# barbararoessle/e2e_multi_view_matching

Hardware: NVIDIA H100
Metric: view-tuples/sec @1024 kpts 5-view (higher is better)
Workload: dtype f32 via split operands on the tensor cores (fp16x3 / tf32x3, fp32-faithful) / f64 pose kernels

## Files before the change

e2e_multi_view_matching_b200/csrc/gemm_tc.cu:

```cuda
#include <cstring>
#include <map>
#include <mutex>
#include <tuple>
#include <cuda_fp16.h>
#include "common.cuh"
#include "kernels.cuh"
#include "tc_common.cuh"

namespace {

constexpr int BM = 128;
constexpr int PRODUCER_WARP = 8;
constexpr int NTHREADS = 384;
constexpr int PRODUCER_REGS = 40, CONSUMER_REGS = 232;
enum { W_RAW = 0, W_TF32 = 1, W_F16 = 2 };

template <int BN, int NPASS, int WM>
struct Cfg {
  static constexpr int BK = WM == W_F16 ? 64 : 32;
  static constexpr int A_BYTES = BM * BK * 4;
  static constexpr int W_PLANE = BN * 128;
  static constexpr int PLANES = NPASS == 3 ? 2 : 1;
  static constexpr int STAGE_BYTES = A_BYTES + PLANES * W_PLANE;
  static constexpr int TMA_BYTES = A_BYTES + (WM == W_RAW ? 1 : PLANES) * W_PLANE;
  static constexpr int STAGES = (196608 / STAGE_BYTES) < 6 ? (196608 / STAGE_BYTES) : 6;
  static constexpr bool STAGED = BN == 128 && NPASS == 3 && WM != W_RAW;
  static constexpr int OUT_BYTES = STAGED ? 2 * 16384 : 0;
  static constexpr int SMEM_BYTES = STAGES * STAGE_BYTES + OUT_BYTES + 1024  + 256 ;
  static_assert(SMEM_BYTES <= 232448, "over the sm_90 dynamic shared memory opt-in limit");
};

struct GArgs {
  const float* bias;
  const float* R; int ldr;
  float* C; int ldc;
  int M, N, K, K1;
  float alpha;
  int relu;
  float* VT; int vt_col0; int n_pad;
  float* KLO; float* VTLO;
  __half* KH16; __half* KL16; __half* VH16; __half* VL16;
  int tiles_m, tiles_n;
  int ksplit;
  int stage;
};

struct StoreMaps {
  CUtensorMap c, r, p[4];
};

struct ScoreTab {
  int n_pairs, batch, n_views, n_pad;
  int a[MVM_MAX_PAIRS], b[MVM_MAX_PAIRS], m[MVM_MAX_PAIRS], n[MVM_MAX_PAIRS];
  float* scores[MVM_MAX_PAIRS];
};

__device__ __forceinline__ float tf32_hi(float x) {
  return __uint_as_float((__float_as_uint(x) + 0x1000u) & 0xffffe000u);
}
__device__ __forceinline__ void split_pack_h(float x0, float x1, uint32_t& hi, uint32_t& lo) {
  const __half2 h = __floats2half2_rn(x0, x1);
  const float2 hf = __half22float2(h);
  const __half2 l = __floats2half2_rn(x0 - hf.x, x1 - hf.y);
  hi = *reinterpret_cast<const uint32_t*>(&h);
  lo = *reinterpret_cast<const uint32_t*>(&l);
}
__device__ __forceinline__ void sts_f2(uint32_t a, float2 v) {
  asm volatile("st.shared.v2.f32 [%0], {%1, %2};" ::"r"(a), "f"(v.x), "f"(v.y) : "memory");
}
__device__ __forceinline__ void sts_u32(uint32_t a, uint32_t v) {
  asm volatile("st.shared.b32 [%0], %1;" ::"r"(a), "r"(v) : "memory");
}
__device__ __forceinline__ float2 lds_f2(uint32_t a) {
  float2 v;
  asm volatile("ld.shared.v2.f32 {%0, %1}, [%2];" : "=f"(v.x), "=f"(v.y) : "r"(a) : "memory");
  return v;
}
__device__ __forceinline__ void fence_afrag(uint32_t (&a)[4][4]) {
#pragma unroll
  for (int i = 0; i < 4; ++i)
#pragma unroll
    for (int e = 0; e < 4; ++e) asm volatile("" : "+r"(a[i][e])::"memory");
}

template <int BN, int NPASS, int WM, bool SCORE>
__global__ void __launch_bounds__(NTHREADS, 1)
gemm_wg_kernel(const __grid_constant__ CUtensorMap tmA, const __grid_constant__ CUtensorMap tmA2,
               const __grid_constant__ CUtensorMap tmWhi, const __grid_constant__ CUtensorMap tmWlo,
               const __grid_constant__ GArgs g, const __grid_constant__ ScoreTab st,
               const __grid_constant__ StoreMaps sm) {
  using C_ = Cfg<BN, NPASS, WM>;
  static_assert(NPASS == 3 || WM == W_RAW, "single pass reads the raw W");
  constexpr int BK = C_::BK, STAGES = C_::STAGES, A_BYTES = C_::A_BYTES, W_PLANE = C_::W_PLANE;
  constexpr int STAGE_BYTES = C_::STAGE_BYTES;
  constexpr int KSTEPS = 4;
  constexpr bool PIPE = BN == 128;
  constexpr bool STAGED = C_::STAGED && !SCORE;
  extern __shared__ uint8_t smem_raw[];
  uint8_t* smem = reinterpret_cast<uint8_t*>((reinterpret_cast<uintptr_t>(smem_raw) + 1023) & ~uintptr_t(1023));
  uint8_t* obuf = smem + STAGES * STAGE_BYTES;
  uint64_t* full = reinterpret_cast<uint64_t*>(obuf + C_::OUT_BYTES);
  uint64_t* empty = full + STAGES;
  uint64_t* ostaged = empty + STAGES;
  uint64_t* ofree = ostaged + 2;

  const int warp = threadIdx.x >> 5, lane = threadIdx.x & 31;
  const int nk = SCORE ? g.K / BK : g.K / BK / g.ksplit;
  const int per_prob = g.tiles_m * g.tiles_n;
  const int n_tiles = SCORE ? per_prob * st.n_pairs * st.batch : per_prob * g.ksplit;
  auto decode = [&](int tile, int& m0, int& n0, int& a_row, int& w_row, int& prob) {
    prob = tile / per_prob;
    const int r = tile % per_prob;
    m0 = (r / g.tiles_n) * BM; n0 = (r % g.tiles_n) * BN;
    if (!SCORE) {
      a_row = m0; w_row = n0;
    } else {
      const int p = prob / st.batch, bi = prob % st.batch;
      a_row = (bi * st.n_views + st.a[p]) * st.n_pad + m0;
      w_row = (bi * st.n_views + st.b[p]) * st.n_pad + n0;
    }
  };
  auto tile_kind = [&](int n0) {
    if (g.VT && n0 >= g.vt_col0) return -1;
    if (g.KH16 && n0 >= 256) return 1;
    if (g.KLO && n0 >= 256 && n0 < 512) return 2;
    return 0;
  };

  if (threadIdx.x == 0) {
    for (int s = 0; s < STAGES; ++s) {
      tc::mbar_init(full + s, 1);
      tc::mbar_init(empty + s, 256);
    }
    if (STAGED)
      for (int b = 0; b < 2; ++b) {
        tc::mbar_init(ostaged + b, 256);
        tc::mbar_init(ofree + b, 1);
      }
    tc::fence_barrier_init();
  }
  __syncthreads();

  if (warp >= PRODUCER_WARP) {
    asm volatile("setmaxnreg.dec.sync.aligned.u32 %0;" ::"n"(PRODUCER_REGS));
    if (STAGED && g.stage && warp == PRODUCER_WARP + 1 && lane == 0) {
      tc::prefetch_tmap(&sm.c);
      if (g.R) tc::prefetch_tmap(&sm.r);
      if (g.KH16)
        for (int i = 0; i < 4; ++i) tc::prefetch_tmap(&sm.p[i]);
      if (g.KLO) tc::prefetch_tmap(&sm.p[0]);
      auto hand_back = [&](uint32_t u, int tile, int q) {
        uint64_t* bar = ofree + (u & 1);
        if (!g.R) {
          tc::mbar_arrive(bar);
        } else if (tile < n_tiles) {
          int m0, n0, a_row, w_row, prob;
          decode(tile, m0, n0, a_row, w_row, prob);
          tc::mbar_arrive_expect_tx(bar, 16384);
          tc::tma_load_2d(obuf + (u & 1) * 16384, &sm.r, bar, n0 + 32 * q, m0);
        }
      };
      hand_back(0, blockIdx.x, 0);
      hand_back(1, blockIdx.x, 1);
      uint32_t u = 0;
      for (int tile = blockIdx.x; tile < n_tiles; tile += gridDim.x) {
        int m0, n0, a_row, w_row, prob;
        decode(tile, m0, n0, a_row, w_row, prob);
        const int kind = tile_kind(n0);
        if (kind < 0) continue;
        const int rounds = kind == 2 ? 8 : 4;
        for (int j = 0; j < rounds; ++j, ++u) {
          const uint8_t* buf = obuf + (u & 1) * 16384;
          tc::mbar_wait(ostaged + (u & 1), (u >> 1) & 1);
          if (kind == 0) {
            tc::tma_store_2d(&sm.c, buf, n0 + 32 * j, m0 + prob * g.tiles_m * BM);
          } else if (kind == 1) {
            const bool v = n0 >= 512;
            tc::tma_store_2d(&sm.p[(v ? 2 : 0) + (j & 1)], buf, n0 - (v ? 512 : 256) + 64 * (j >> 1), m0);
          } else {
            if (j & 1) tc::tma_store_2d(&sm.p[0], buf, n0 - 256 + 32 * (j >> 1), m0);
            else tc::tma_store_2d(&sm.c, buf, n0 + 32 * (j >> 1), m0);
          }
          tc::tma_store_commit();
          tc::tma_store_wait_read<0>();
          hand_back(u + 2, j < 2 ? tile : tile + gridDim.x, (j + 2) & 3);
        }
      }
      tc::tma_store_wait_all();
    }
    if (warp == PRODUCER_WARP && lane == 0) {
      tc::prefetch_tmap(&tmA); tc::prefetch_tmap(&tmA2); tc::prefetch_tmap(&tmWhi); tc::prefetch_tmap(&tmWlo);
      uint32_t it = 0;
      for (int tile = blockIdx.x; tile < n_tiles; tile += gridDim.x) {
        int m0, n0, a_row, w_row, prob;
        decode(tile, m0, n0, a_row, w_row, prob);
        for (int kt = 0; kt < nk; ++kt, ++it) {
          const int s = it % STAGES;
          tc::mbar_wait(empty + s, ((it / STAGES) & 1) ^ 1);
          tc::mbar_arrive_expect_tx(full + s, C_::TMA_BYTES);
          uint8_t* sp = smem + s * STAGE_BYTES;
          const int k = kt * BK + (SCORE ? 0 : prob * nk * BK);
          if (k < g.K1) tc::tma_load_2d(sp, &tmA, full + s, k, a_row);
          else tc::tma_load_2d(sp, &tmA2, full + s, k - g.K1, a_row);
          if (WM == W_F16) {
            if (k < g.K1) tc::tma_load_2d(sp + 16384, &tmA, full + s, k + 32, a_row);
            else tc::tma_load_2d(sp + 16384, &tmA2, full + s, k + 32 - g.K1, a_row);
          }
          tc::tma_load_2d(sp + A_BYTES, &tmWhi, full + s, k, w_row);
          if (WM != W_RAW) tc::tma_load_2d(sp + A_BYTES + W_PLANE, &tmWlo, full + s, k, w_row);
        }
      }
    }
    return;
  }

  asm volatile("setmaxnreg.inc.sync.aligned.u32 %0;" ::"n"(CONSUMER_REGS));
  const int wg = warp >> 2, wq = warp & 3;
  const int gr = lane >> 2, tq = lane & 3;
  const int row0 = wg * 64 + wq * 16 + gr;
  float acc[BN / 2];
  uint32_t ahi0[KSTEPS][4], alo0[KSTEPS][4], ahi1[KSTEPS][4], alo1[KSTEPS][4];

  auto prep = [&](uint32_t it, uint32_t (&ahi)[KSTEPS][4], uint32_t (&alo)[KSTEPS][4]) {
      const int s = it % STAGES;
      tc::mbar_wait(full + s, (it / STAGES) & 1);
      uint8_t* sp = smem + s * STAGE_BYTES;
      if (WM == W_RAW && NPASS == 3) {
        float4* w = reinterpret_cast<float4*>(sp + A_BYTES);
        float4* wl = reinterpret_cast<float4*>(sp + A_BYTES + W_PLANE);
#pragma unroll 4
        for (int i = threadIdx.x; i < BN * 32 / 4; i += 256) {
          const float4 x = w[i];
          float4 h;
          h.x = tc::tf32_rn(x.x); h.y = tc::tf32_rn(x.y); h.z = tc::tf32_rn(x.z); h.w = tc::tf32_rn(x.w);
          w[i] = h;
          wl[i] = make_float4(tc::tf32_rn(x.x - h.x), tc::tf32_rn(x.y - h.y), tc::tf32_rn(x.z - h.z), tc::tf32_rn(x.w - h.w));
        }
// ... 3 lines not shown
      const uint8_t* ar = sp + row0 * 128;
#pragma unroll
      for (int kk = 0; kk < KSTEPS; ++kk) {
        if (WM == W_F16) {
          const uint8_t* ab = ar + (kk >> 1) * 16384;
          const int ch = 4 * (kk & 1) + (tq >> 1), wo = (tq & 1) * 8;
          const float2 x0 = *reinterpret_cast<const float2*>(ab + ((ch ^ gr) << 4) + wo);
          const float2 x1 = *reinterpret_cast<const float2*>(ab + 1024 + ((ch ^ gr) << 4) + wo);
          const float2 x2 = *reinterpret_cast<const float2*>(ab + (((ch + 2) ^ gr) << 4) + wo);
          const float2 x3 = *reinterpret_cast<const float2*>(ab + 1024 + (((ch + 2) ^ gr) << 4) + wo);
          split_pack_h(x0.x, x0.y, ahi[kk][0], alo[kk][0]);
          split_pack_h(x1.x, x1.y, ahi[kk][1], alo[kk][1]);
          split_pack_h(x2.x, x2.y, ahi[kk][2], alo[kk][2]);
          split_pack_h(x3.x, x3.y, ahi[kk][3], alo[kk][3]);
        } else {
          float x[4];
          x[0] = *reinterpret_cast<const float*>(ar + (((2 * kk) ^ gr) << 4) + tq * 4);
          x[1] = *reinterpret_cast<const float*>(ar + 1024 + (((2 * kk) ^ gr) << 4) + tq * 4);
          x[2] = *reinterpret_cast<const float*>(ar + (((2 * kk + 1) ^ gr) << 4) + tq * 4);
          x[3] = *reinterpret_cast<const float*>(ar + 1024 + (((2 * kk + 1) ^ gr) << 4) + tq * 4);
#pragma unroll
          for (int e = 0; e < 4; ++e) {
            if (NPASS == 3) {
              const float h = tf32_hi(x[e]);
              ahi[kk][e] = __float_as_uint(h);
              alo[kk][e] = __float_as_uint(tf32_hi(x[e] - h));
            } else {
              ahi[kk][e] = __float_as_uint(x[e]);
            }
          }
        }
      }
  };
  auto issue = [&](uint32_t it, const uint32_t (&ahi)[KSTEPS][4], const uint32_t (&alo)[KSTEPS][4]) {
      const uint32_t whi = tc::smem_u32(smem + (it % STAGES) * STAGE_BYTES + A_BYTES);
      tc::wgmma_fence();
#pragma unroll
      for (int kk = 0; kk < KSTEPS; ++kk) {
#pragma unroll
        for (int nh = 0; nh < BN / 128; ++nh) {
          float* d = acc + nh * 64;
          const uint32_t wb = whi + nh * 16384 + kk * 32;
          if (WM == W_F16) {
            tc::wgmma_f16_rs<128, 0>(d, ahi[kk], tc::make_sw128_desc(wb));
            tc::wgmma_f16_rs<128, 0>(d, ahi[kk], tc::make_sw128_desc(wb + W_PLANE));
            tc::wgmma_f16_rs<128, 0>(d, alo[kk], tc::make_sw128_desc(wb));
          } else {
            tc::wgmma_tf32_rs<128>(d, ahi[kk], tc::make_sw128_desc(wb));
            if (NPASS == 3) {
              tc::wgmma_tf32_rs<128>(d, ahi[kk], tc::make_sw128_desc(wb + W_PLANE));
              tc::wgmma_tf32_rs<128>(d, alo[kk], tc::make_sw128_desc(wb));
            }
          }
        }
      }
      tc::wgmma_commit();
  };
  auto keep = [&](uint32_t (&ahi)[KSTEPS][4], uint32_t (&alo)[KSTEPS][4]) {
    fence_afrag(ahi);
    if (NPASS == 3) fence_afrag(alo);
  };

  auto stage_round = [&](uint32_t u, int n0, int i0, int ni, int mode, int plane) {
    const uint32_t buf = tc::smem_u32(obuf + (u & 1) * 16384);
    float2 bv[8];
#pragma unroll
    for (int c = 0; c < ni; ++c) {
      const int n = n0 + 8 * (i0 + c) + 2 * tq;
      bv[c] = g.bias ? make_float2(__ldg(g.bias + n), __ldg(g.bias + n + 1)) : make_float2(0.f, 0.f);
    }
    tc::mbar_wait(ofree + (u & 1), (u >> 1) & 1);
#pragma unroll
    for (int c = 0; c < ni; ++c) {
      const int i = i0 + c;
#pragma unroll
      for (int hh = 0; hh < 2; ++hh) {
        const int r = row0 + 8 * hh;
        float x0 = __fmul_rn(g.alpha, acc[4 * i + 2 * hh]), x1 = __fmul_rn(g.alpha, acc[4 * i + 2 * hh + 1]);
        if (g.bias) { x0 = __fadd_rn(x0, bv[c].x); x1 = __fadd_rn(x1, bv[c].y); }
// ... 50 lines not shown
        prep(it + kt, ahi0, alo0);
        issue(it + kt, ahi0, alo0);
        tc::wgmma_wait<0>();
        tc::fence_acc<BN>(acc);
        keep(ahi0, alo0);
        tc::mbar_arrive(empty + (it + kt) % STAGES);
      }
    }
    it += nk;

    if (SCORE) {
      const int p = prob / st.batch, bi = prob % st.batch;
      const int pm = st.m[p], pn = st.n[p];
      float* Cp = st.scores[p] + (long long)bi * (pm + 1) * (pn + 1);
#pragma unroll
      for (int hh = 0; hh < 2; ++hh) {
        const int gm = m0 + row0 + 8 * hh;
        if (gm >= pm) continue;
#pragma unroll
        for (int i = 0; i < BN / 8; ++i) {
          const int gn = n0 + 8 * i + 2 * tq;
          if (gn < pn) Cp[(long long)gm * (pn + 1) + gn] = g.alpha * acc[4 * i + 2 * hh];
          if (gn + 1 < pn) Cp[(long long)gm * (pn + 1) + gn + 1] = g.alpha * acc[4 * i + 2 * hh + 1];
        }
      }
      continue;
    }
    if constexpr (STAGED) {
      const int kind = g.stage ? tile_kind(n0) : -1;
      if (kind >= 0) {
#pragma unroll
        for (int j = 0; j < 8; ++j) {
          if (kind == 1) {
            if (j < 4) stage_round(u + j, n0, 8 * (j >> 1), 8, 1, j & 1);
          } else if (kind == 2) {
            stage_round(u + j, n0, 4 * (j >> 1), 4, 2, j & 1);
          } else if (j < 4) {
            stage_round(u + j, n0, 4 * j, 4, 0, 0);
          }
        }
        u += kind == 2 ? 8 : 4;
        continue;
      }
    }
    auto put = [&](int m, int n, float x0, float x1) {
      if (g.VT && n >= g.vt_col0) {
        const int slab = m / g.n_pad, ii = m % g.n_pad;
        const long long off = ((long long)slab * (g.N - g.vt_col0) + (n - g.vt_col0)) * g.n_pad + ii;
        if (g.VTLO) {
          const float h0 = tf32_hi(x0), h1 = tf32_hi(x1);
          g.VT[off] = h0; g.VT[off + g.n_pad] = h1;
          g.VTLO[off] = tf32_hi(x0 - h0); g.VTLO[off + g.n_pad] = tf32_hi(x1 - h1);
        } else {
          g.VT[off] = x0; g.VT[off + g.n_pad] = x1;
        }
      } else if (g.KH16 && n >= 256) {
        const bool is_v = n >= 512;
        const long long o = (long long)m * 256 + n - (is_v ? 512 : 256);
        uint32_t hi, lo;
        split_pack_h(x0, x1, hi, lo);
        *reinterpret_cast<uint32_t*>((is_v ? g.VH16 : g.KH16) + o) = hi;
        *reinterpret_cast<uint32_t*>((is_v ? g.VL16 : g.KL16) + o) = lo;
      } else if (g.KLO && n >= 256 && n < 512) {
        const float h0 = tf32_hi(x0), h1 = tf32_hi(x1);
        *reinterpret_cast<float2*>(g.C + (long long)m * g.ldc + n) = make_float2(h0, h1);
        *reinterpret_cast<float2*>(g.KLO + (long long)m * 256 + n - 256) = make_float2(tf32_hi(x0 - h0), tf32_hi(x1 - h1));
      } else {
        const long long c_row = m + (long long)prob * g.tiles_m * BM;
        *reinterpret_cast<float2*>(g.C + c_row * g.ldc + n) = make_float2(x0, x1);
      }
    };
    if constexpr (PIPE) {
      constexpr int ICH = 8;
#pragma unroll
// ... 15 lines not shown
          const int i = i0 + c, n = n0 + 8 * i + 2 * tq;
#pragma unroll
          for (int hh = 0; hh < 2; ++hh) {
            const int m = m0 + row0 + 8 * hh;
            if (m >= g.M) continue;
            float x0 = g.alpha * acc[4 * i + 2 * hh], x1 = g.alpha * acc[4 * i + 2 * hh + 1];
            if (g.bias) { x0 += bv[c].x; x1 += bv[c].y; }
            if (g.relu) { x0 = fmaxf(x0, 0.f); x1 = fmaxf(x1, 0.f); }
            if (g.R) { x0 += rv[c][hh].x; x1 += rv[c][hh].y; }
            put(m, n, x0, x1);
          }
        }
      }
    } else {
#pragma unroll
      for (int hh = 0; hh < 2; ++hh) {
        const int m = m0 + row0 + 8 * hh;
        if (m >= g.M) continue;
#pragma unroll
        for (int i = 0; i < BN / 8; ++i) {
          const int n = n0 + 8 * i + 2 * tq;
          float x0 = g.alpha * acc[4 * i + 2 * hh], x1 = g.alpha * acc[4 * i + 2 * hh + 1];
          if (g.bias) { x0 += __ldg(g.bias + n); x1 += __ldg(g.bias + n + 1); }
          if (g.relu) { x0 = fmaxf(x0, 0.f); x1 = fmaxf(x1, 0.f); }
          if (g.R) {
            const float2 r = __ldg(reinterpret_cast<const float2*>(g.R + (long long)m * g.ldr + n));
            x0 += r.x; x1 += r.y;
          }
          put(m, n, x0, x1);
        }
      }
    }
  }
}

template <int BN, int NPASS, int WM, bool SCORE>
int launch_wg(const CUtensorMap* tA, const CUtensorMap* tA2, const CUtensorMap* tWhi, const CUtensorMap* tWlo,
              const GArgs& g, const ScoreTab& st, long long n_tiles, bool persistent, cudaStream_t stream,
              const StoreMaps& sm) {
  using C_ = Cfg<BN, NPASS, WM>;
  if (!tA || !tA2 || !tWhi || !tWlo) return MVM_ERR_LAUNCH;
  if (n_tiles <= 0) return MVM_OK;
  if (cudaFuncSetAttribute(gemm_wg_kernel<BN, NPASS, WM, SCORE>, cudaFuncAttributeMaxDynamicSharedMemorySize,
                           C_::SMEM_BYTES) != cudaSuccess)
    return MVM_ERR_LAUNCH;
  const int n_sm = mvm_dev_info().n_sm;
  const int grid = (persistent && n_tiles > n_sm) ? n_sm : (int)n_tiles;
  gemm_wg_kernel<BN, NPASS, WM, SCORE><<<grid, NTHREADS, C_::SMEM_BYTES, stream>>>(*tA, *tA2, *tWhi, *tWlo, g, st, sm);
  MVM_CHECK_LAUNCH();
  return MVM_OK;
}

StoreMaps no_store_maps() {
  StoreMaps none;
  memset(&none, 0, sizeof(none));
  return none;
}

GArgs make_args(const GemmDesc& d, float* VT, int vt_col0, int n_pad, float* KLO, float* VTLO, int bn) {
  GArgs g;
  memset(&g, 0, sizeof(g));
  g.bias = d.bias; g.R = d.R; g.ldr = d.ldr; g.C = d.C; g.ldc = d.ldc; g.M = d.M; g.N = d.N; g.K = d.K;
  g.K1 = d.K1; g.alpha = d.alpha; g.relu = d.relu; g.VT = VT; g.vt_col0 = vt_col0; g.n_pad = n_pad;
  g.KLO = KLO; g.VTLO = VTLO;
  g.tiles_m = mvm_div_up(d.M, BM); g.tiles_n = d.N / bn; g.ksplit = 1;
  return g;
// ... 61 lines not shown

}

const CUtensorMap* mvm_get_tmap_3d(const float* base, long long slabs, long long rows, long long cols,
                                   long long ld_row, long long ld_slab, int box_rows) {
  std::lock_guard<std::mutex> lk(g_tmap_mu);
  TmKey key(base, slabs, rows, cols, ld_row, ld_slab, box_rows);
  auto it = g_tmaps.find(key);
  if (it != g_tmaps.end()) return it->second;
  EncodeFn enc = get_encode();
  if (!enc) return nullptr;
  CUtensorMap* tm = new CUtensorMap;
  const int rank = slabs > 0 ? 3 : 2;
  cuuint64_t dims[3] = {(cuuint64_t)cols, (cuuint64_t)rows, (cuuint64_t)(slabs > 0 ? slabs : 1)};
  cuuint64_t strides[2] = {(cuuint64_t)ld_row * 4, (cuuint64_t)ld_slab * 4};
  cuuint32_t box[3] = {32, (cuuint32_t)box_rows, 1};
  cuuint32_t estr[3] = {1, 1, 1};
  CUresult r = enc(tm, CU_TENSOR_MAP_DATA_TYPE_FLOAT32, rank, const_cast<float*>(base), dims, strides, box, estr,
                   CU_TENSOR_MAP_INTERLEAVE_NONE, CU_TENSOR_MAP_SWIZZLE_128B, CU_TENSOR_MAP_L2_PROMOTION_L2_128B,
                   CU_TENSOR_MAP_FLOAT_OOB_FILL_NONE);
  if (r != CUDA_SUCCESS) {
    fprintf(stderr, "[mvm_b200] cuTensorMapEncodeTiled failed (%d) rows=%lld cols=%lld ld=%lld\n", (int)r, rows, cols, ld_row);
    delete tm;
    return nullptr;
  }
  g_tmaps[key] = tm;
  return tm;
}

const CUtensorMap* mvm_get_tmap_2d(const float* base, long long rows, long long cols, long long ld, int box_rows) {
  return mvm_get_tmap_3d(base, 0, rows, cols, ld, 0, box_rows);
}

const CUtensorMap* mvm_get_tmap_2d_f16(const void* base, long long rows, long long cols, long long ld, int box_rows) {
  std::lock_guard<std::mutex> lk(g_tmap_mu);
  TmKey key(base, -16, rows, cols, ld, 0, box_rows);
  auto it = g_tmaps.find(key);
  if (it != g_tmaps.end()) return it->second;
  EncodeFn enc = get_encode();
  if (!enc) return nullptr;
  CUtensorMap* tm = new CUtensorMap;
  cuuint64_t dims[2] = {(cuuint64_t)cols, (cuuint64_t)rows};
  cuuint64_t strides[1] = {(cuuint64_t)ld * 2};
  cuuint32_t box[2] = {64, (cuuint32_t)box_rows};
  cuuint32_t estr[2] = {1, 1};
  CUresult r = enc(tm, CU_TENSOR_MAP_DATA_TYPE_FLOAT16, 2, const_cast<void*>(base), dims, strides, box, estr,
                   CU_TENSOR_MAP_INTERLEAVE_NONE, CU_TENSOR_MAP_SWIZZLE_128B, CU_TENSOR_MAP_L2_PROMOTION_L2_128B,
                   CU_TENSOR_MAP_FLOAT_OOB_FILL_NONE);
  if (r != CUDA_SUCCESS) {
    fprintf(stderr, "[mvm_b200] cuTensorMapEncodeTiled (f16) failed (%d) rows=%lld cols=%lld ld=%lld\n", (int)r, rows, cols, ld);
    delete tm;
    return nullptr;
  }
  g_tmaps[key] = tm;
  return tm;
}


int g_gemm_bn = 256;
extern "C" void mvm_debug_set_gemm_tile(int bn) { g_gemm_bn = bn == 256 ? 256 : 128; }
int g_gemm_persist = 1;
extern "C" void mvm_debug_set_gemm_kernel(int persistent) { g_gemm_persist = persistent ? 1 : 0; }

int mvm_default_gemm_tile() { return g_gemm_bn; }
int mvm_default_gemm_persistent() { return g_gemm_persist; }

int launch_gemm_tc(const GemmDesc& d, int n_pass, float* VT, int vt_col0, int n_pad, cudaStream_t stream,
                   float* KLO, float* VTLO, int gemm_tile, int gemm_persist) {
  if (gemm_tile < 0) gemm_tile = g_gemm_bn;
  if (gemm_persist < 0) gemm_persist = g_gemm_persist;
  MVM_REQUIRE(gemm_desc_valid(d, GEMM_TC_TF32));
  MVM_REQUIRE(d.W || (n_pass == 3 && d.Whi && d.Wlo));
  MVM_REQUIRE(mvm_aligned(KLO, 8));
  MvmProfScope prof__(MVM_TAG_GEMM, stream);
  if (gemm_persist && n_pass == 3 && d.Whi && d.Wlo) return launch_gemm_tc_persist(d, VT, vt_col0, n_pad, KLO, VTLO, stream);
  if (gemm_tile == 256 && d.N % 256 == 0) {
    if (n_pass == 3 && d.Whi && d.Wlo) return launch_cfg<256, 3, W_TF32>(d, VT, vt_col0, n_pad, KLO, VTLO, false, stream);
    if (n_pass == 1) return launch_cfg<256, 1, W_RAW>(d, VT, vt_col0, n_pad, nullptr, nullptr, false, stream);
  }
  if (n_pass == 3 && d.Whi && d.Wlo) return launch_cfg<128, 3, W_TF32>(d, VT, vt_col0, n_pad, KLO, VTLO, false, stream);
  if (n_pass == 3) return launch_cfg<128, 3, W_RAW>(d, VT, vt_col0, n_pad, KLO, VTLO, false, stream);
  return launch_cfg<128, 1, W_RAW>(d, VT, vt_col0, n_pad, nullptr, nullptr, false, stream);
}

int launch_gemm_tc_persist(const GemmDesc& d, float* VT, int vt_col0, int n_pad, float* KLO, float* VTLO,
                           cudaStream_t stream, const HalfPlanes* hp, int ksplit, float* slabs) {
  MVM_REQUIRE(ksplit >= 1 && (ksplit == 1 || (slabs && d.M % BM == 0 && d.K % (32 * ksplit) == 0 && !d.Whi16 && !d.bias && !d.R && !d.A2 &&
                                               !d.relu && !VT && !KLO && !hp)));
  const bool f16 = d.Whi16 != nullptr && d.Wlo16 != nullptr && d.K % 64 == 0 && d.K1 % 64 == 0 && d.wscale > 0.f;
  MVM_REQUIRE(f16 ? gemm_desc_valid(d, GEMM_TC_F16) : gemm_desc_valid(d, GEMM_TC_TF32) && d.Whi && d.Wlo);
  MVM_REQUIRE(mvm_aligned(KLO, 8) && mvm_aligned(slabs, 16));
  MVM_REQUIRE(!hp || (mvm_aligned(hp->kh, 4) && mvm_aligned(hp->kl, 4) && mvm_aligned(hp->vh, 4) && mvm_aligned(hp->vl, 4)));
  const CUtensorMap* tA = mvm_get_tmap_2d(d.A, d.M, d.K1, d.lda, BM);
  const CUtensorMap* tA2 = d.A2 ? mvm_get_tmap_2d(d.A2, d.M, d.K - d.K1, d.lda2, BM) : tA;
  GArgs g = make_args(d, VT, vt_col0, n_pad, KLO, VTLO, 128);
  if (ksplit > 1) { g.C = slabs; g.ldc = d.N; }
  g.ksplit = ksplit;
  if (hp) {
    g.KH16 = (__half*)hp->kh; g.KL16 = (__half*)hp->kl; g.VH16 = (__half*)hp->vh; g.VL16 = (__half*)hp->vl;
  }
  const long long n_tiles = (long long)g.tiles_m * g.tiles_n * ksplit;
  StoreMaps sm = no_store_maps();
  const void* planes[4] = {g.KH16, g.KL16, g.VH16, g.VL16};
  bool stage = mvm_aligned(g.C, 16) && mvm_aligned(g.R, 16) && mvm_aligned(g.KLO, 16) && (!g.VT || g.vt_col0 % 128 == 0) &&
               (!g.R || (!g.KH16 && !g.KLO && !g.VT));
  for (const void* p : planes) stage = stage && mvm_aligned(p, 16);
  if (stage) {
    const CUtensorMap* c = mvm_get_tmap_2d(g.C, (long long)(ksplit - 1) * g.tiles_m * BM + g.M, g.N, g.ldc, BM);
    const CUtensorMap* r = g.R ? mvm_get_tmap_2d(g.R, g.M, g.N, g.ldr, BM) : c;
    if (!c || !r) return MVM_ERR_LAUNCH;
    sm.c = *c; sm.r = *r;
    for (int i = 0; i < 4; ++i) {
      const CUtensorMap* p = g.KH16 ? mvm_get_tmap_2d_f16(planes[i], g.M, 256, 256, BM)
                                    : g.KLO && i == 0 ? mvm_get_tmap_2d(g.KLO, g.M, 256, 256, BM) : c;
      if (!p) return MVM_ERR_LAUNCH;
      sm.p[i] = *p;
    }
    g.stage = 1;
  }
  if (f16) {
    g.alpha = d.alpha / d.wscale;
    const CUtensorMap* tWhi = mvm_get_tmap_2d_f16(d.Whi16, d.N, d.K, d.ldw, 128);
    const CUtensorMap* tWlo = mvm_get_tmap_2d_f16(d.Wlo16, d.N, d.K, d.ldw, 128);
    return launch_wg<128, 3, W_F16, false>(tA, tA2, tWhi, tWlo, g, no_scores(), n_tiles, true, stream, sm);
  }
  const CUtensorMap* tWhi = mvm_get_tmap_2d(d.Whi, d.N, d.K, d.ldw, 128);
  const CUtensorMap* tWlo = mvm_get_tmap_2d(d.Wlo, d.N, d.K, d.ldw, 128);
  return launch_wg<128, 3, W_TF32, false>(tA, tA2, tWhi, tWlo, g, no_scores(), n_tiles, true, stream, sm);
}

int launch_splitk_reduce(const float* slabs, float* C, int M, int N, int ldc, int ksplit, cudaStream_t stream) {
  MVM_REQUIRE(N % 4 == 0 && ldc % 4 == 0 && mvm_aligned(slabs, 16) && mvm_aligned(C, 16));
  const long long n = (long long)M * (N / 4);
  splitk_reduce_kernel<<<(unsigned)((n + 255) / 256), 256, 0, stream>>>(reinterpret_cast<const float4*>(slabs), C, M, N / 4, ldc, ksplit);
  MVM_CHECK_LAUNCH();
  return MVM_OK;
}

int launch_score_gemm_tc(const float* mdesc, float* hi, float* lo, int n_pad, const PairTable& tab, int batch,
                         float alpha, cudaStream_t stream) {
  MvmProfScope prof__(MVM_TAG_SCORE, stream);
  const int n_sm = mvm_dev_info().n_sm;
  const long long rows = (long long)batch * tab.n_views * n_pad;
  split_planes_kernel<<<n_sm * 4, 256, 0, stream>>>(reinterpret_cast<const float4*>(mdesc), reinterpret_cast<float4*>(hi),
                                                    reinterpret_cast<float4*>(lo), rows * 256 / 4);
  MVM_CHECK_LAUNCH();
  const CUtensorMap* tA = mvm_get_tmap_2d(mdesc, rows, 256, 256, BM);
  const CUtensorMap* tWhi = mvm_get_tmap_2d(hi, rows, 256, 256, 128);
  const CUtensorMap* tWlo = mvm_get_tmap_2d(lo, rows, 256, 256, 128);
  ScoreTab st = no_scores();
  st.n_pairs = tab.n_pairs; st.batch = batch; st.n_views = tab.n_views; st.n_pad = n_pad;
  int max_m = 0, max_n = 0;
  for (int p = 0; p < tab.n_pairs; ++p) {
    st.a[p] = tab.a[p]; st.b[p] = tab.b[p]; st.m[p] = tab.m[p]; st.n[p] = tab.n[p]; st.scores[p] = tab.scores[p];
// ... 11 lines not shown
```

e2e_multi_view_matching_b200/csrc/tc_common.cuh:

```cuda
#pragma once
#include <cuda.h>
#include <cuda_runtime.h>
#include <stdint.h>

namespace tc {

__device__ __forceinline__ uint32_t smem_u32(const void* p) {
  return static_cast<uint32_t>(__cvta_generic_to_shared(p));
}

__device__ __forceinline__ void mbar_init(uint64_t* bar, uint32_t count) {
  asm volatile("mbarrier.init.shared::cta.b64 [%0], %1;" ::"r"(smem_u32(bar)), "r"(count));
}
__device__ __forceinline__ void fence_barrier_init() {
  asm volatile("fence.mbarrier_init.release.cluster;" ::: "memory");
}
__device__ __forceinline__ void fence_proxy_async() {
  asm volatile("fence.proxy.async.shared::cta;" ::: "memory");
}
__device__ __forceinline__ void mbar_arrive_expect_tx(uint64_t* bar, uint32_t bytes) {
  asm volatile("mbarrier.arrive.expect_tx.shared::cta.b64 _, [%0], %1;" ::"r"(smem_u32(bar)), "r"(bytes)
               : "memory");
}
__device__ __forceinline__ void mbar_arrive(uint64_t* bar) {
// ... 21 lines not shown
  asm volatile(
      "cp.async.bulk.tensor.2d.shared::cluster.global.tile.mbarrier::complete_tx::bytes [%0], [%1, {%3, %4}], [%2];"
      ::"r"(smem_u32(dst)), "l"(reinterpret_cast<uint64_t>(m)), "r"(smem_u32(bar)), "r"(c0), "r"(c1)
      : "memory");
}
__device__ __forceinline__ void tma_load_3d(void* dst, const CUtensorMap* m, uint64_t* bar, int c0, int c1,
                                            int c2) {
  asm volatile(
      "cp.async.bulk.tensor.3d.shared::cluster.global.tile.mbarrier::complete_tx::bytes [%0], [%1, {%3, %4, %5}], [%2];"
      ::"r"(smem_u32(dst)), "l"(reinterpret_cast<uint64_t>(m)), "r"(smem_u32(bar)), "r"(c0), "r"(c1), "r"(c2)
      : "memory");
}

__device__ __forceinline__ void tma_store_2d(const CUtensorMap* m, const void* src, int c0, int c1) {
  asm volatile("cp.async.bulk.tensor.2d.global.shared::cta.tile.bulk_group [%0, {%2, %3}], [%1];"
               ::"l"(reinterpret_cast<uint64_t>(m)), "r"(smem_u32(src)), "r"(c0), "r"(c1)
               : "memory");
}
__device__ __forceinline__ void tma_store_commit() { asm volatile("cp.async.bulk.commit_group;" ::: "memory"); }
template <int N>
__device__ __forceinline__ void tma_store_wait_read() {
  asm volatile("cp.async.bulk.wait_group.read %0;" ::"n"(N) : "memory");
}
__device__ __forceinline__ void tma_store_wait_all() { asm volatile("cp.async.bulk.wait_group 0;" ::: "memory"); }

__device__ __forceinline__ uint64_t make_sw128_desc(uint32_t smem_addr) {
  uint64_t d = 0;
  d |= static_cast<uint64_t>((smem_addr & 0x3FFFF) >> 4);
  d |= static_cast<uint64_t>(1) << 16;
  d |= static_cast<uint64_t>(1024 >> 4) << 32;
  d |= static_cast<uint64_t>(1) << 62;
  return d;
}
__device__ __forceinline__ void wgmma_fence() { asm volatile("wgmma.fence.sync.aligned;" ::: "memory"); }
__device__ __forceinline__ void wgmma_commit() { asm volatile("wgmma.commit_group.sync.aligned;" ::: "memory"); }
template <int N>
__device__ __forceinline__ void wgmma_wait() { asm volatile("wgmma.wait_group.sync.aligned %0;" ::"n"(N) : "memory"); }
template <int N>
__device__ __forceinline__ void fence_acc(float* d) {
#pragma unroll
  for (int i = 0; i < N / 2; ++i) asm volatile("" : "+f"(d[i])::"memory");
}

template <int N> __device__ __forceinline__ void wgmma_tf32_rs(float* d, const uint32_t* a, uint64_t bdesc);
template <int N, int TB> __device__ __forceinline__ void wgmma_f16_rs(float* d, const uint32_t* a, uint64_t bdesc);
template <> __device__ __forceinline__ void wgmma_tf32_rs<64>(float* d, const uint32_t* a, uint64_t bdesc) {
  asm volatile(
      "{\n\t.reg .pred p;\n\tsetp.eq.u32 p, 1, 1;\n\t"
      "wgmma.mma_async.sync.aligned.m64n64k8.f32.tf32.tf32 "
      "{%0, %1, %2, %3, %4, %5, %6, %7, %8, %9, %10, %11, %12, %13, %14, %15, %16, %17, %18, %19, %20, %21, %22, %23, %24, %25, %26, %27, %28, %29, %30, %31}, {%32, %33, %34, %35}, %36, p, 1, 1;\n\t}"
      : "+f"(d[0]), "+f"(d[1]), "+f"(d[2]), "+f"(d[3]), "+f"(d[4]), "+f"(d[5]), "+f"(d[6]), "+f"(d[7]), "+f"(d[8]), "+f"(d[9]), "+f"(d[10]), "+f"(d[11]), "+f"(d[12]), "+f"(d[13]), "+f"(d[14]), "+f"(d[15]), "+f"(d[16]), "+f"(d[17]), "+f"(d[18]), "+f"(d[19]), "+f"(d[20]), "+f"(d[21]), "+f"(d[22]), "+f"(d[23]), "+f"(d[24]), "+f"(d[25]), "+f"(d[26]), "+f"(d[27]), "+f"(d[28]), "+f"(d[29]), "+f"(d[30]), "+f"(d[31])
      : "r"(a[0]), "r"(a[1]), "r"(a[2]), "r"(a[3]), "l"(bdesc));
}
template <> __device__ __forceinline__ void wgmma_f16_rs<64, 0>(float* d, const uint32_t* a, uint64_t bdesc) {
  asm volatile(
      "{\n\t.reg .pred p;\n\tsetp.eq.u32 p, 1, 1;\n\t"
      "wgmma.mma_async.sync.aligned.m64n64k16.f32.f16.f16 "
      "{%0, %1, %2, %3, %4, %5, %6, %7, %8, %9, %10, %11, %12, %13, %14, %15, %16, %17, %18, %19, %20, %21, %22, %23, %24, %25, %26, %27, %28, %29, %30, %31}, {%32, %33, %34, %35}, %36, p, 1, 1, 0;\n\t}"
      : "+f"(d[0]), "+f"(d[1]), "+f"(d[2]), "+f"(d[3]), "+f"(d[4]), "+f"(d[5]), "+f"(d[6]), "+f"(d[7]), "+f"(d[8]), "+f"(d[9]), "+f"(d[10]), "+f"(d[11]), "+f"(d[12]), "+f"(d[13]), "+f"(d[14]), "+f"(d[15]), "+f"(d[16]), "+f"(d[17]), "+f"(d[18]), "+f"(d[19]), "+f"(d[20]), "+f"(d[21]), "+f"(d[22]), "+f"(d[23]), "+f"(d[24]), "+f"(d[25]), "+f"(d[26]), "+f"(d[27]), "+f"(d[28]), "+f"(d[29]), "+f"(d[30]), "+f"(d[31])
      : "r"(a[0]), "r"(a[1]), "r"(a[2]), "r"(a[3]), "l"(bdesc));
}
template <> __device__ __forceinline__ void wgmma_f16_rs<64, 1>(float* d, const uint32_t* a, uint64_t bdesc) {
  asm volatile(
      "{\n\t.reg .pred p;\n\tsetp.eq.u32 p, 1, 1;\n\t"
      "wgmma.mma_async.sync.aligned.m64n64k16.f32.f16.f16 "
      "{%0, %1, %2, %3, %4, %5, %6, %7, %8, %9, %10, %11, %12, %13, %14, %15, %16, %17, %18, %19, %20, %21, %22, %23, %24, %25, %26, %27, %28, %29, %30, %31}, {%32, %33, %34, %35}, %36, p, 1, 1, 1;\n\t}"
// ... 4 lines not shown
  asm volatile(
      "{\n\t.reg .pred p;\n\tsetp.eq.u32 p, 1, 1;\n\t"
      "wgmma.mma_async.sync.aligned.m64n128k8.f32.tf32.tf32 "
      "{%0, %1, %2, %3, %4, %5, %6, %7, %8, %9, %10, %11, %12, %13, %14, %15, %16, %17, %18, %19, %20, %21, %22, %23, %24, %25, %26, %27, %28, %29, %30, %31, %32, %33, %34, %35, %36, %37, %38, %39, %40, %41, %42, %43, %44, %45, %46, %47, %48, %49, %50, %51, %52, %53, %54, %55, %56, %57, %58, %59, %60, %61, %62, %63}, {%64, %65, %66, %67}, %68, p, 1, 1;\n\t}"
      : "+f"(d[0]), "+f"(d[1]), "+f"(d[2]), "+f"(d[3]), "+f"(d[4]), "+f"(d[5]), "+f"(d[6]), "+f"(d[7]), "+f"(d[8]), "+f"(d[9]), "+f"(d[10]), "+f"(d[11]), "+f"(d[12]), "+f"(d[13]), "+f"(d[14]), "+f"(d[15]), "+f"(d[16]), "+f"(d[17]), "+f"(d[18]), "+f"(d[19]), "+f"(d[20]), "+f"(d[21]), "+f"(d[22]), "+f"(d[23]), "+f"(d[24]), "+f"(d[25]), "+f"(d[26]), "+f"(d[27]), "+f"(d[28]), "+f"(d[29]), "+f"(d[30]), "+f"(d[31]), "+f"(d[32]), "+f"(d[33]), "+f"(d[34]), "+f"(d[35]), "+f"(d[36]), "+f"(d[37]), "+f"(d[38]), "+f"(d[39]), "+f"(d[40]), "+f"(d[41]), "+f"(d[42]), "+f"(d[43]), "+f"(d[44]), "+f"(d[45]), "+f"(d[46]), "+f"(d[47]), "+f"(d[48]), "+f"(d[49]), "+f"(d[50]), "+f"(d[51]), "+f"(d[52]), "+f"(d[53]), "+f"(d[54]), "+f"(d[55]), "+f"(d[56]), "+f"(d[57]), "+f"(d[58]), "+f"(d[59]), "+f"(d[60]), "+f"(d[61]), "+f"(d[62]), "+f"(d[63])
      : "r"(a[0]), "r"(a[1]), "r"(a[2]), "r"(a[3]), "l"(bdesc));
}
template <> __device__ __forceinline__ void wgmma_f16_rs<128, 0>(float* d, const uint32_t* a, uint64_t bdesc) {
  asm volatile(
      "{\n\t.reg .pred p;\n\tsetp.eq.u32 p, 1, 1;\n\t"
      "wgmma.mma_async.sync.aligned.m64n128k16.f32.f16.f16 "
      "{%0, %1, %2, %3, %4, %5, %6, %7, %8, %9, %10, %11, %12, %13, %14, %15, %16, %17, %18, %19, %20, %21, %22, %23, %24, %25, %26, %27, %28, %29, %30, %31, %32, %33, %34, %35, %36, %37, %38, %39, %40, %41, %42, %43, %44, %45, %46, %47, %48, %49, %50, %51, %52, %53, %54, %55, %56, %57, %58, %59, %60, %61, %62, %63}, {%64, %65, %66, %67}, %68, p, 1, 1, 0;\n\t}"
      : "+f"(d[0]), "+f"(d[1]), "+f"(d[2]), "+f"(d[3]), "+f"(d[4]), "+f"(d[5]), "+f"(d[6]), "+f"(d[7]), "+f"(d[8]), "+f"(d[9]), "+f"(d[10]), "+f"(d[11]), "+f"(d[12]), "+f"(d[13]), "+f"(d[14]), "+f"(d[15]), "+f"(d[16]), "+f"(d[17]), "+f"(d[18]), "+f"(d[19]), "+f"(d[20]), "+f"(d[21]), "+f"(d[22]), "+f"(d[23]), "+f"(d[24]), "+f"(d[25]), "+f"(d[26]), "+f"(d[27]), "+f"(d[28]), "+f"(d[29]), "+f"(d[30]), "+f"(d[31]), "+f"(d[32]), "+f"(d[33]), "+f"(d[34]), "+f"(d[35]), "+f"(d[36]), "+f"(d[37]), "+f"(d[38]), "+f"(d[39]), "+f"(d[40]), "+f"(d[41]), "+f"(d[42]), "+f"(d[43]), "+f"(d[44]), "+f"(d[45]), "+f"(d[46]), "+f"(d[47]), "+f"(d[48]), "+f"(d[49]), "+f"(d[50]), "+f"(d[51]), "+f"(d[52]), "+f"(d[53]), "+f"(d[54]), "+f"(d[55]), "+f"(d[56]), "+f"(d[57]), "+f"(d[58]), "+f"(d[59]), "+f"(d[60]), "+f"(d[61]), "+f"(d[62]), "+f"(d[63])
      : "r"(a[0]), "r"(a[1]), "r"(a[2]), "r"(a[3]), "l"(bdesc));
}
template <> __device__ __forceinline__ void wgmma_f16_rs<128, 1>(float* d, const uint32_t* a, uint64_t bdesc) {
  asm volatile(
      "{\n\t.reg .pred p;\n\tsetp.eq.u32 p, 1, 1;\n\t"
      "wgmma.mma_async.sync.aligned.m64n128k16.f32.f16.f16 "
      "{%0, %1, %2, %3, %4, %5, %6, %7, %8, %9, %10, %11, %12, %13, %14, %15, %16, %17, %18, %19, %20, %21, %22, %23, %24, %25, %26, %27, %28, %29, %30, %31, %32, %33, %34, %35, %36, %37, %38, %39, %40, %41, %42, %43, %44, %45, %46, %47, %48, %49, %50, %51, %52, %53, %54, %55, %56, %57, %58, %59, %60, %61, %62, %63}, {%64, %65, %66, %67}, %68, p, 1, 1, 1;\n\t}"
      : "+f"(d[0]), "+f"(d[1]), "+f"(d[2]), "+f"(d[3]), "+f"(d[4]), "+f"(d[5]), "+f"(d[6]), "+f"(d[7]), "+f"(d[8]), "+f"(d[9]), "+f"(d[10]), "+f"(d[11]), "+f"(d[12]), "+f"(d[13]), "+f"(d[14]), "+f"(d[15]), "+f"(d[16]), "+f"(d[17]), "+f"(d[18]), "+f"(d[19]), "+f"(d[20]), "+f"(d[21]), "+f"(d[22]), "+f"(d[23]), "+f"(d[24]), "+f"(d[25]), "+f"(d[26]), "+f"(d[27]), "+f"(d[28]), "+f"(d[29]), "+f"(d[30]), "+f"(d[31]), "+f"(d[32]), "+f"(d[33]), "+f"(d[34]), "+f"(d[35]), "+f"(d[36]), "+f"(d[37]), "+f"(d[38]), "+f"(d[39]), "+f"(d[40]), "+f"(d[41]), "+f"(d[42]), "+f"(d[43]), "+f"(d[44]), "+f"(d[45]), "+f"(d[46]), "+f"(d[47]), "+f"(d[48]), "+f"(d[49]), "+f"(d[50]), "+f"(d[51]), "+f"(d[52]), "+f"(d[53]), "+f"(d[54]), "+f"(d[55]), "+f"(d[56]), "+f"(d[57]), "+f"(d[58]), "+f"(d[59]), "+f"(d[60]), "+f"(d[61]), "+f"(d[62]), "+f"(d[63])
      : "r"(a[0]), "r"(a[1]), "r"(a[2]), "r"(a[3]), "l"(bdesc));
}

__device__ __forceinline__ float tf32_rn(float x) {
  uint32_t r;
  asm("cvt.rna.tf32.f32 %0, %1;" : "=r"(r) : "f"(x));
  return __uint_as_float(r);
}

}

const CUtensorMap* mvm_get_tmap_2d(const float* base, long long rows, long long cols, long long ld, int box_rows);
const CUtensorMap* mvm_get_tmap_2d_f16(const void* base, long long rows, long long cols, long long ld, int box_rows);

const CUtensorMap* mvm_get_tmap_3d(const float* base, long long slabs, long long rows, long long cols,
                                   long long ld_row, long long ld_slab, int box_rows);
```

Baseline: 217.4.

## Add wide 128x256 fp16x3 GEMM tile variant with BK=32 and 64B swizzle

Adds a second persistent warp-specialized GEMM kernel that uses 256-column output tiles with a K-depth of 32 and 64-byte swizzled fp16 W planes. It is selected for staged, non-split, plain-output GEMMs whose N is a multiple of 256. The kernel body is refactored into a template shared by both configurations, and the output staging rounds, TMA f16 tensor maps and wgmma descriptors are generalised to the new tile shape. Wider tiles are meant to improve reuse of the A operand and cut per-tile overhead, at the cost of fewer tiles to spread across SMs, a shallower K step per stage, and new swizzle/descriptor logic that could be wrong.

```diff
diff --git a/e2e_multi_view_matching_b200/csrc/gemm_tc.cu b/e2e_multi_view_matching_b200/csrc/gemm_tc.cu
--- a/e2e_multi_view_matching_b200/csrc/gemm_tc.cu
+++ b/e2e_multi_view_matching_b200/csrc/gemm_tc.cu
@@ -14,18 +14,35 @@
 constexpr int NTHREADS = 384;
 constexpr int PRODUCER_REGS = 40, CONSUMER_REGS = 232;
 enum { W_RAW = 0, W_TF32 = 1, W_F16 = 2 };
+constexpr int WIDE_BK = 32;
 
 template <int BN, int NPASS, int WM>
 struct Cfg {
   static constexpr int BK = WM == W_F16 ? 64 : 32;
   static constexpr int A_BYTES = BM * BK * 4;
-  static constexpr int W_PLANE = BN * 128;
+  static constexpr int W_ROW = 128;
+  static constexpr int W_PLANE = BN * W_ROW;
   static constexpr int PLANES = NPASS == 3 ? 2 : 1;
   static constexpr int STAGE_BYTES = A_BYTES + PLANES * W_PLANE;
   static constexpr int TMA_BYTES = A_BYTES + (WM == W_RAW ? 1 : PLANES) * W_PLANE;
   static constexpr int STAGES = (196608 / STAGE_BYTES) < 6 ? (196608 / STAGE_BYTES) : 6;
   static constexpr bool STAGED = BN == 128 && NPASS == 3 && WM != W_RAW;
   static constexpr int OUT_BYTES = STAGED ? 2 * 16384 : 0;
+  static constexpr int SMEM_BYTES = STAGES * STAGE_BYTES + OUT_BYTES + 1024  + 256 ;
+  static_assert(SMEM_BYTES <= 232448, "over the sm_90 dynamic shared memory opt-in limit");
+  static constexpr bool PIPE = BN == 128;
+};
+
+struct WideCfg {
+  static constexpr int BN = 256, BK = WIDE_BK;
+  static constexpr int A_BYTES = BM * BK * 4;
+  static constexpr int W_ROW = BK * 2;
+  static constexpr int W_PLANE = BN * W_ROW;
+  static constexpr int STAGE_BYTES = A_BYTES + 2 * W_PLANE;
+  static constexpr int TMA_BYTES = STAGE_BYTES;
+  static constexpr int STAGES = 196608 / STAGE_BYTES;
+  static constexpr bool STAGED = true, PIPE = true;
+  static constexpr int OUT_BYTES = 2 * 16384;
   static constexpr int SMEM_BYTES = STAGES * STAGE_BYTES + OUT_BYTES + 1024  + 256 ;
   static_assert(SMEM_BYTES <= 232448, "over the sm_90 dynamic shared memory opt-in limit");
 };
@@ -76,25 +93,24 @@
   asm volatile("ld.shared.v2.f32 {%0, %1}, [%2];" : "=f"(v.x), "=f"(v.y) : "r"(a) : "memory");
   return v;
 }
-__device__ __forceinline__ void fence_afrag(uint32_t (&a)[4][4]) {
-#pragma unroll
-  for (int i = 0; i < 4; ++i)
+template <int KSTEPS>
+__device__ __forceinline__ void fence_afrag(uint32_t (&a)[KSTEPS][4]) {
+#pragma unroll
+  for (int i = 0; i < KSTEPS; ++i)
 #pragma unroll
     for (int e = 0; e < 4; ++e) asm volatile("" : "+r"(a[i][e])::"memory");
 }
 
-template <int BN, int NPASS, int WM, bool SCORE>
-__global__ void __launch_bounds__(NTHREADS, 1)
-gemm_wg_kernel(const __grid_constant__ CUtensorMap tmA, const __grid_constant__ CUtensorMap tmA2,
-               const __grid_constant__ CUtensorMap tmWhi, const __grid_constant__ CUtensorMap tmWlo,
-               const __grid_constant__ GArgs g, const __grid_constant__ ScoreTab st,
-               const __grid_constant__ StoreMaps sm) {
-  using C_ = Cfg<BN, NPASS, WM>;
+template <class C_, int BN, int NPASS, int WM, bool SCORE>
+__device__ __forceinline__ void gemm_wg_body(const CUtensorMap& tmA, const CUtensorMap& tmA2, const CUtensorMap& tmWhi,
+                                             const CUtensorMap& tmWlo, const GArgs& g, const ScoreTab& st,
+                                             const StoreMaps& sm) {
   static_assert(NPASS == 3 || WM == W_RAW, "single pass reads the raw W");
   constexpr int BK = C_::BK, STAGES = C_::STAGES, A_BYTES = C_::A_BYTES, W_PLANE = C_::W_PLANE;
   constexpr int STAGE_BYTES = C_::STAGE_BYTES;
-  constexpr int KSTEPS = 4;
-  constexpr bool PIPE = BN == 128;
+  constexpr int KSTEPS = WM == W_F16 ? BK / 16 : BK / 8;
+  constexpr bool PIPE = C_::PIPE;
+  constexpr int ROUNDS = BN / 32;
   constexpr bool STAGED = C_::STAGED && !SCORE;
   extern __shared__ uint8_t smem_raw[];
   uint8_t* smem = reinterpret_cast<uint8_t*>((reinterpret_cast<uintptr_t>(smem_raw) + 1023) & ~uintptr_t(1023));
@@ -123,7 +139,7 @@
   auto tile_kind = [&](int n0) {
     if (g.VT && n0 >= g.vt_col0) return -1;
     if (g.KH16 && n0 >= 256) return 1;
-    if (g.KLO && n0 >= 256 && n0 < 512) return 2;
+    if (BN == 128 && g.KLO && n0 >= 256 && n0 < 512) return 2;
     return 0;
   };
 
@@ -168,7 +184,7 @@
         decode(tile, m0, n0, a_row, w_row, prob);
         const int kind = tile_kind(n0);
         if (kind < 0) continue;
-        const int rounds = kind == 2 ? 8 : 4;
+        const int rounds = kind == 2 ? 8 : ROUNDS;
         for (int j = 0; j < rounds; ++j, ++u) {
           const uint8_t* buf = obuf + (u & 1) * 16384;
           tc::mbar_wait(ostaged + (u & 1), (u >> 1) & 1);
@@ -183,7 +199,7 @@
           }
           tc::tma_store_commit();
           tc::tma_store_wait_read<0>();
-          hand_back(u + 2, j < 2 ? tile : tile + gridDim.x, (j + 2) & 3);
+          hand_back(u + 2, j < ROUNDS - 2 ? tile : tile + gridDim.x, (j + 2) & (ROUNDS - 1));
         }
       }
       tc::tma_store_wait_all();
@@ -202,7 +218,7 @@
           const int k = kt * BK + (SCORE ? 0 : prob * nk * BK);
           if (k < g.K1) tc::tma_load_2d(sp, &tmA, full + s, k, a_row);
           else tc::tma_load_2d(sp, &tmA2, full + s, k - g.K1, a_row);
-          if (WM == W_F16) {
+          if (WM == W_F16 && BK == 64) {
             if (k < g.K1) tc::tma_load_2d(sp + 16384, &tmA, full + s, k + 32, a_row);
             else tc::tma_load_2d(sp + 16384, &tmA2, full + s, k + 32 - g.K1, a_row);
           }
@@ -272,6 +288,7 @@
         }
       }
   };
+  auto wdesc = [](uint32_t a) { return C_::W_ROW == 128 ? tc::make_sw128_desc(a) : tc::make_sw64_desc(a); };
   auto issue = [&](uint32_t it, const uint32_t (&ahi)[KSTEPS][4], const uint32_t (&alo)[KSTEPS][4]) {
       const uint32_t whi = tc::smem_u32(smem + (it % STAGES) * STAGE_BYTES + A_BYTES);
       tc::wgmma_fence();
@@ -280,11 +297,11 @@
 #pragma unroll
         for (int nh = 0; nh < BN / 128; ++nh) {
           float* d = acc + nh * 64;
-          const uint32_t wb = whi + nh * 16384 + kk * 32;
+          const uint32_t wb = whi + nh * 128 * C_::W_ROW + kk * 32;
           if (WM == W_F16) {
-            tc::wgmma_f16_rs<128, 0>(d, ahi[kk], tc::make_sw128_desc(wb));
-            tc::wgmma_f16_rs<128, 0>(d, ahi[kk], tc::make_sw128_desc(wb + W_PLANE));
-            tc::wgmma_f16_rs<128, 0>(d, alo[kk], tc::make_sw128_desc(wb));
+            tc::wgmma_f16_rs<128, 0>(d, ahi[kk], wdesc(wb));
+            tc::wgmma_f16_rs<128, 0>(d, ahi[kk], wdesc(wb + W_PLANE));
+            tc::wgmma_f16_rs<128, 0>(d, alo[kk], wdesc(wb));
           } else {
             tc::wgmma_tf32_rs<128>(d, ahi[kk], tc::make_sw128_desc(wb));
             if (NPASS == 3) {
@@ -401,14 +418,14 @@
 #pragma unroll
         for (int j = 0; j < 8; ++j) {
           if (kind == 1) {
-            if (j < 4) stage_round(u + j, n0, 8 * (j >> 1), 8, 1, j & 1);
-          } else if (kind == 2) {
+            if (j < ROUNDS) stage_round(u + j, n0, 8 * (j >> 1), 8, 1, j & 1);
+          } else if (BN == 128 && kind == 2) {
             stage_round(u + j, n0, 4 * (j >> 1), 4, 2, j & 1);
-          } else if (j < 4) {
+          } else if (j < ROUNDS) {
             stage_round(u + j, n0, 4 * j, 4, 0, 0);
           }
         }
-        u += kind == 2 ? 8 : 4;
+        u += kind == 2 ? 8 : ROUNDS;
         continue;
       }
     }
@@ -490,6 +507,23 @@
       }
     }
   }
+}
+
+template <int BN, int NPASS, int WM, bool SCORE>
+__global__ void __launch_bounds__(NTHREADS, 1)
+gemm_wg_kernel(const __grid_constant__ CUtensorMap tmA, const __grid_constant__ CUtensorMap tmA2,
+               const __grid_constant__ CUtensorMap tmWhi, const __grid_constant__ CUtensorMap tmWlo,
+               const __grid_constant__ GArgs g, const __grid_constant__ ScoreTab st,
+               const __grid_constant__ StoreMaps sm) {
+  gemm_wg_body<Cfg<BN, NPASS, WM>, BN, NPASS, WM, SCORE>(tmA, tmA2, tmWhi, tmWlo, g, st, sm);
+}
+
+__global__ void __launch_bounds__(NTHREADS, 1)
+gemm_wg_kernel_wide(const __grid_constant__ CUtensorMap tmA, const __grid_constant__ CUtensorMap tmA2,
+                    const __grid_constant__ CUtensorMap tmWhi, const __grid_constant__ CUtensorMap tmWlo,
+                    const __grid_constant__ GArgs g, const __grid_constant__ ScoreTab st,
+                    const __grid_constant__ StoreMaps sm) {
+  gemm_wg_body<WideCfg, 256, 3, W_F16, false>(tmA, tmA2, tmWhi, tmWlo, g, st, sm);
 }
 
 template <int BN, int NPASS, int WM, bool SCORE>
@@ -617,9 +651,11 @@
   return mvm_get_tmap_3d(base, 0, rows, cols, ld, 0, box_rows);
 }
 
-const CUtensorMap* mvm_get_tmap_2d_f16(const void* base, long long rows, long long cols, long long ld, int box_rows) {
+const CUtensorMap* mvm_get_tmap_2d_f16(const void* base, long long rows, long long cols, long long ld, int box_rows,
+                                       int box_cols) {
+  if (box_cols != 64 && box_cols != 32) return nullptr;
   std::lock_guard<std::mutex> lk(g_tmap_mu);
-  TmKey key(base, -16, rows, cols, ld, 0, box_rows);
+  TmKey key(base, -16, rows, cols, ld, box_cols, box_rows);
   auto it = g_tmaps.find(key);
   if (it != g_tmaps.end()) return it->second;
   EncodeFn enc = get_encode();
@@ -627,10 +663,10 @@
   CUtensorMap* tm = new CUtensorMap;
   cuuint64_t dims[2] = {(cuuint64_t)cols, (cuuint64_t)rows};
   cuuint64_t strides[1] = {(cuuint64_t)ld * 2};
-  cuuint32_t box[2] = {64, (cuuint32_t)box_rows};
+  cuuint32_t box[2] = {(cuuint32_t)box_cols, (cuuint32_t)box_rows};
   cuuint32_t estr[2] = {1, 1};
   CUresult r = enc(tm, CU_TENSOR_MAP_DATA_TYPE_FLOAT16, 2, const_cast<void*>(base), dims, strides, box, estr,
-                   CU_TENSOR_MAP_INTERLEAVE_NONE, CU_TENSOR_MAP_SWIZZLE_128B, CU_TENSOR_MAP_L2_PROMOTION_L2_128B,
+                   CU_TENSOR_MAP_INTERLEAVE_NONE, box_cols == 64 ? CU_TENSOR_MAP_SWIZZLE_128B : CU_TENSOR_MAP_SWIZZLE_64B, CU_TENSOR_MAP_L2_PROMOTION_L2_128B,
                    CU_TENSOR_MAP_FLOAT_OOB_FILL_NONE);
   if (r != CUDA_SUCCESS) {
     fprintf(stderr, "[mvm_b200] cuTensorMapEncodeTiled (f16) failed (%d) rows=%lld cols=%lld ld=%lld\n", (int)r, rows, cols, ld);
@@ -666,6 +702,10 @@
   if (n_pass == 3 && d.Whi && d.Wlo) return launch_cfg<128, 3, W_TF32>(d, VT, vt_col0, n_pad, KLO, VTLO, false, stream);
   if (n_pass == 3) return launch_cfg<128, 3, W_RAW>(d, VT, vt_col0, n_pad, KLO, VTLO, false, stream);
   return launch_cfg<128, 1, W_RAW>(d, VT, vt_col0, n_pad, nullptr, nullptr, false, stream);
+}
+
+bool use_wide_tiles(const GArgs& g, int ksplit) {
+  return g.stage && ksplit == 1 && !g.KLO && !g.VT && g.N % 256 == 0;
 }
 
 int launch_gemm_tc_persist(const GemmDesc& d, float* VT, int vt_col0, int n_pad, float* KLO, float* VTLO,
@@ -705,6 +745,21 @@
   }
   if (f16) {
     g.alpha = d.alpha / d.wscale;
+    if (use_wide_tiles(g, ksplit)) {
+      g.tiles_n = g.N / 256;
+      const CUtensorMap* tWhi = mvm_get_tmap_2d_f16(d.Whi16, d.N, d.K, d.ldw, 256, WideCfg::W_ROW / 2);
+      const CUtensorMap* tWlo = mvm_get_tmap_2d_f16(d.Wlo16, d.N, d.K, d.ldw, 256, WideCfg::W_ROW / 2);
+      if (!tWhi || !tWlo) return MVM_ERR_LAUNCH;
+      if (cudaFuncSetAttribute(gemm_wg_kernel_wide, cudaFuncAttributeMaxDynamicSharedMemorySize, WideCfg::SMEM_BYTES) !=
+          cudaSuccess)
+        return MVM_ERR_LAUNCH;
+      const long long tiles = (long long)g.tiles_m * g.tiles_n;
+      const int n_sm = mvm_dev_info().n_sm;
+      gemm_wg_kernel_wide<<<(int)(tiles < n_sm ? tiles : n_sm), NTHREADS, WideCfg::SMEM_BYTES, stream>>>(
+          *tA, *tA2, *tWhi, *tWlo, g, no_scores(), sm);
+      MVM_CHECK_LAUNCH();
+      return MVM_OK;
+    }
     const CUtensorMap* tWhi = mvm_get_tmap_2d_f16(d.Whi16, d.N, d.K, d.ldw, 128);
     const CUtensorMap* tWlo = mvm_get_tmap_2d_f16(d.Wlo16, d.N, d.K, d.ldw, 128);
     return launch_wg<128, 3, W_F16, false>(tA, tA2, tWhi, tWlo, g, no_scores(), n_tiles, true, stream, sm);
diff --git a/e2e_multi_view_matching_b200/csrc/tc_common.cuh b/e2e_multi_view_matching_b200/csrc/tc_common.cuh
--- a/e2e_multi_view_matching_b200/csrc/tc_common.cuh
+++ b/e2e_multi_view_matching_b200/csrc/tc_common.cuh
@@ -77,6 +77,14 @@
   d |= static_cast<uint64_t>(1) << 62;
   return d;
 }
+__device__ __forceinline__ uint64_t make_sw64_desc(uint32_t smem_addr) {
+  uint64_t d = 0;
+  d |= static_cast<uint64_t>((smem_addr & 0x3FFFF) >> 4);
+  d |= static_cast<uint64_t>(1) << 16;
+  d |= static_cast<uint64_t>(512 >> 4) << 32;
+  d |= static_cast<uint64_t>(2) << 62;
+  return d;
+}
 __device__ __forceinline__ void wgmma_fence() { asm volatile("wgmma.fence.sync.aligned;" ::: "memory"); }
 __device__ __forceinline__ void wgmma_commit() { asm volatile("wgmma.commit_group.sync.aligned;" ::: "memory"); }
 template <int N>
@@ -147,7 +155,8 @@
 }
 
 const CUtensorMap* mvm_get_tmap_2d(const float* base, long long rows, long long cols, long long ld, int box_rows);
-const CUtensorMap* mvm_get_tmap_2d_f16(const void* base, long long rows, long long cols, long long ld, int box_rows);
+const CUtensorMap* mvm_get_tmap_2d_f16(const void* base, long long rows, long long cols, long long ld, int box_rows,
+                                       int box_cols = 64);
 
 const CUtensorMap* mvm_get_tmap_3d(const float* base, long long slabs, long long rows, long long cols,
                                    long long ld_row, long long ld_slab, int box_rows);
```

After: 220.7, median of 6. 1.01x the previous value.
